# FasterDecoding/TEAL

Measured on AMD Instinct MI355X. Metric: decode tokens/sec (bs=1), Llama-2-7B fp16 @50% activation sparsity, higher is better.
Workload: dtype f16; 1 GPU; Llama-2-7B bs=1 decode, uniform 50% sparsity, hipGraph-captured step; mode=engine, parallelism=single GPU, context_positions=6..866

## Files before the change

### teal_amd/csrc/teal_sampler.hip

```cpp
#include "teal_common.h"

namespace teal {


template <bool BF16>
__device__ __forceinline__ void sample_full(const uint16_t* __restrict__ logits, const int V, const int top_k,
                                            const float inv_temp, unsigned long long* __restrict__ rng_state,
                                            int* __restrict__ token_out, int* __restrict__ pos_inout,
                                            int* __restrict__ history, const int history_len) {
    __shared__ unsigned int hist[256];
    __shared__ unsigned int whist[16][256];
    __shared__ float fred[16];
    __shared__ int ired[16];
    __shared__ unsigned int sel[2];
    __shared__ unsigned int suf[256];
    const int tid = threadIdx.x, lane = tid & 63, wave = tid >> 6;
    const bool filter = top_k > 0 && top_k < V;
    const int V8 = V >> 3;
    const u32x4* lv = reinterpret_cast<const u32x4*>(logits);
    uint32_t pivot_key = 0;
    float mx = -INFINITY;
    for (int i = tid; i < 16 * 256; i += 1024) (&whist[0][0])[i] = 0;
    __syncthreads();
    for (int i = tid; i < V8; i += 1024) {
        const u32x4 w = lv[i];
#pragma unroll
        for (int j = 0; j < 4; ++j) {
            const uint32_t lo = w[j] & 0xFFFFu, hi = w[j] >> 16;
            mx = fmaxf(mx, fmaxf(bits_to_float(lo, BF16), bits_to_float(hi, BF16)));
            if (filter) {
                atomicAdd(&whist[wave][order_key16(lo, BF16) >> 8], 1u);
                atomicAdd(&whist[wave][order_key16(hi, BF16) >> 8], 1u);
            }
        }
    }
    for (int i = (V8 << 3) + tid; i < V; i += 1024) {
        mx = fmaxf(mx, bits_to_float(logits[i], BF16));
        if (filter) atomicAdd(&whist[wave][order_key16(logits[i], BF16) >> 8], 1u);
    }
#pragma unroll
    for (int d = 32; d >= 1; d >>= 1) mx = fmaxf(mx, __shfl_xor(mx, d));
    if (lane == 0) fred[wave] = mx;
    __syncthreads();
    if (tid < 256) {
        unsigned int a = 0;
#pragma unroll
        for (int w = 0; w < 16; ++w) a += whist[w][tid];
        hist[tid] = a;
    }
    __syncthreads();
    mx = fred[0];
#pragma unroll
    for (int w = 1; w < 16; ++w) mx = fmaxf(mx, fred[w]);
    if (filter) {
        select_bin(hist, suf, sel, (unsigned int)top_k, tid);
        __syncthreads();
        const unsigned int hb = sel[0], need2 = sel[1];
        __syncthreads();
        for (int i = tid; i < 16 * 256; i += 1024) (&whist[0][0])[i] = 0;
        __syncthreads();
        for (int i = tid; i < V8; i += 1024) {
            const u32x4 w = lv[i];
#pragma unroll
            for (int j = 0; j < 4; ++j) {
                const uint32_t k0 = order_key16(w[j] & 0xFFFFu, BF16), k1 = order_key16(w[j] >> 16, BF16);
                if ((k0 >> 8) == hb) atomicAdd(&whist[wave][k0 & 0xFFu], 1u);
                if ((k1 >> 8) == hb) atomicAdd(&whist[wave][k1 & 0xFFu], 1u);
            }
        }
        for (int i = (V8 << 3) + tid; i < V; i += 1024) {
            const uint32_t k = order_key16(logits[i], BF16);
            if ((k >> 8) == hb) atomicAdd(&whist[wave][k & 0xFFu], 1u);
        }
        __syncthreads();
        if (tid < 256) {
            unsigned int a = 0;
#pragma unroll
            for (int w = 0; w < 16; ++w) a += whist[w][tid];
            hist[tid] = a;
        }
        __syncthreads();
        select_bin(hist, suf, sel, need2, tid);
        if (tid == 0) sel[0] = (hb << 8) | sel[0];
        __syncthreads();
        pivot_key = sel[0];
    }
    const uint32_t seed = (uint32_t)rng_state[0], ctr = (uint32_t)rng_state[1];
    float best = -1.0f;
    int besti = 0x7FFFFFFF;
    auto consider = [&](const uint32_t b, const int i) {
        if (filter && order_key16(b, BF16) < pivot_key) return;
        const float pnum = expf((bits_to_float(b, BF16) - mx) * inv_temp);
        const float u = ((float)(hash3(seed, ctr, (uint32_t)i) >> 8) + 0.5f) * (1.0f / 16777216.0f);
        const float scv = pnum / (-logf(u));
        if (scv > best || (scv == best && i < besti)) { best = scv; besti = i; }
    };
    for (int i = tid; i < V8; i += 1024) {
        const u32x4 w = lv[i];
#pragma unroll
        for (int j = 0; j < 4; ++j) {
            consider(w[j] & 0xFFFFu, i * 8 + 2 * j);
            consider(w[j] >> 16, i * 8 + 2 * j + 1);
        }
    }
    for (int i = (V8 << 3) + tid; i < V; i += 1024) consider(logits[i], i);
#pragma unroll
    for (int d = 32; d >= 1; d >>= 1) {
        const float ob = __shfl_xor(best, d);
        const int oi = __shfl_xor(besti, d);
        if (ob > best || (ob == best && oi < besti)) { best = ob; besti = oi; }
    }
    __syncthreads();
    if (lane == 0) { fred[wave] = best; ired[wave] = besti; }
    __syncthreads();
    if (tid == 0) {
        for (int w = 1; w < 16; ++w)
            if (fred[w] > best || (fred[w] == best && ired[w] < besti)) { best = fred[w]; besti = ired[w]; }
        token_out[0] = besti;
        const unsigned long long c = rng_state[1];
        if (history && (long long)c < (long long)history_len) history[c] = besti;
        rng_state[1] = c + 1ull;
        if (pos_inout) pos_inout[0] = pos_inout[0] + 1;
    }
}

template <bool BF16>
__global__ __launch_bounds__(1024) void sample_topk_kernel(const uint16_t* __restrict__ logits, const int V,
                                                            const int top_k, const float inv_temp,
                                                            unsigned long long* __restrict__ rng_state,
                                                            int* __restrict__ token_out, int* __restrict__ pos_inout,
                                                            int* __restrict__ history, const int history_len) {
    sample_full<BF16>(logits, V, top_k, inv_temp, rng_state, token_out, pos_inout, history, history_len);
}

__device__ __forceinline__ bool slot_off(const int* __restrict__ active, const int slot) { return !((active[0] >> slot) & 1); }

template <bool BF16>
__global__ __launch_bounds__(1024) void sample_topk_slot_kernel(const uint16_t* __restrict__ logits, const int V,
                                                                 const int top_k, const float inv_temp,
                                                                 unsigned long long* __restrict__ rng_state,
                                                                 int* __restrict__ token_out, int* __restrict__ pos_inout,
                                                                 int* __restrict__ history, const int history_len,
                                                                 const int* __restrict__ active, const int slot) {
    if (slot_off(active, slot)) return;
    sample_full<BF16>(logits, V, top_k, inv_temp, rng_state, token_out, pos_inout, history, history_len);
}


template <bool BF16, int NV>
__device__ __forceinline__ void sample_window_body(const uint16_t* __restrict__ logits, const int V, const int top_k, const float inv_temp,
                                                   unsigned long long* __restrict__ rng_state, int* __restrict__ token_out,
                                                   int* __restrict__ pos_inout, int* __restrict__ history, const int history_len,
                                                   unsigned long long* __restrict__ phase) {
    auto stamp_s = [&](const int i) { if (phase && threadIdx.x == 0) phase[i] = wall_clock64(); };
    stamp_s(0);
    __shared__ unsigned int hist[256];
    __shared__ unsigned int whist[16][256];
    __shared__ float fred[16];
    __shared__ int ired[16];
    __shared__ unsigned int sel[2];
    const int tid = threadIdx.x, lane = tid & 63, wave = tid >> 6;
    const bool filter = top_k > 0 && top_k < V;
    const int V8 = V >> 3;
    const u32x4* lv = reinterpret_cast<const u32x4*>(logits);
    u32x4 kv[NV];
#pragma unroll
    for (int v = 0; v < NV; ++v) kv[v] = lv[min(v * 1024 + tid, V8 - 1)];
    const unsigned long long seed64 = rng_state[0], ctr64 = rng_state[1];
    const int pos0 = pos_inout ? pos_inout[0] : 0;
    for (int i = tid; i < 16 * 256; i += 1024) (&whist[0][0])[i] = 0;
    uint32_t kmax = 0u;
#pragma unroll
    for (int v = 0; v < NV; ++v) {
        const bool ok = v * 1024 + tid < V8;
#pragma unroll
        for (int j = 0; j < 4; ++j) {
            const uint32_t k0 = order_key16(kv[v][j] & 0xFFFFu, BF16), k1 = order_key16(kv[v][j] >> 16, BF16);
            kv[v][j] = ok ? (k0 | (k1 << 16)) : 0u;
            kmax = ok ? max(kmax, max(k0, k1)) : kmax;
        }
    }
#pragma unroll
    for (int d = 32; d >= 1; d >>= 1) kmax = max(kmax, (uint32_t)__shfl_xor((int)kmax, d));
    if (lane == 0) ired[wave] = (int)kmax;
    __syncthreads();
    kmax = (uint32_t)ired[0];
#pragma unroll
    for (int w = 1; w < 16; ++w) kmax = max(kmax, (uint32_t)ired[w]);
    auto key_bits = [](const uint32_t k) -> uint32_t { return (k & 0x8000u) ? (k ^ 0x8000u) : (~k & 0xFFFFu); };
    const float mx = bits_to_float(key_bits(kmax), BF16);
    stamp_s(1);
    auto merge_hist = [&]() {
        __syncthreads();
        if (tid < 256) {
            unsigned int a = 0;
#pragma unroll
            for (int w = 0; w < 16; ++w) a += whist[w][tid];
            hist[tid] = a;
        }
        __syncthreads();
    };
    uint32_t pivot_key = 0u;
    if (filter) {
        for (int sh = BF16 ? 0 : 3;; sh += 3) {
            if (sh > 8) sh = 8;
#pragma unroll
            for (int v = 0; v < NV; ++v) {
                if (v * 1024 + tid < V8) {
#pragma unroll
                    for (int j = 0; j < 4; ++j) {
                        const uint32_t d0 = (kmax - (kv[v][j] & 0xFFFFu)) >> sh, d1 = (kmax - (kv[v][j] >> 16)) >> sh;
                        if (d0 < 256u) atomicAdd(&whist[wave][255u - d0], 1u);
                        if (d1 < 256u) atomicAdd(&whist[wave][255u - d1], 1u);
                    }
                }
            }
            merge_hist();
            unsigned int inwin = 0;
            {
                unsigned int a = (tid < 256) ? hist[tid] : 0u;
                a = (unsigned int)wave_sum_f((float)a);
                if (lane == 0) fred[wave] = (float)a;
                __syncthreads();
                inwin = (unsigned int)(fred[0] + fred[1] + fred[2] + fred[3]);
            }
            if (inwin >= (unsigned int)top_k || sh == 8) {
                select_bin(hist, nullptr, sel, (unsigned int)top_k, tid);
                const unsigned int d = 255u - sel[0], need2 = sel[1];
                __syncthreads();
                if (sh == 0) {
                    pivot_key = kmax - d;
                } else {
                    for (int i = tid; i < 16 * 256; i += 1024) (&whist[0][0])[i] = 0;
                    __syncthreads();
                    const uint32_t lowmask = (1u << sh) - 1u;
#pragma unroll
                    for (int v = 0; v < NV; ++v) {
                        if (v * 1024 + tid < V8) {
#pragma unroll
                            for (int j = 0; j < 4; ++j) {
                                const uint32_t e0 = kmax - (kv[v][j] & 0xFFFFu), e1 = kmax - (kv[v][j] >> 16);
                                if ((e0 >> sh) == d) atomicAdd(&whist[wave][255u - (e0 & lowmask)], 1u);
                                if ((e1 >> sh) == d) atomicAdd(&whist[wave][255u - (e1 & lowmask)], 1u);
                            }
                        }
                    }
                    merge_hist();
                    select_bin(hist, nullptr, sel, need2, tid);
                    pivot_key = kmax - ((d << sh) | (255u - sel[0]));
                    __syncthreads();
                }
                break;
            }
            for (int i = tid; i < 16 * 256; i += 1024) (&whist[0][0])[i] = 0;
            __syncthreads();
        }
    }
    stamp_s(2);
    const uint32_t seed = (uint32_t)seed64, ctr = (uint32_t)ctr64;
    float best = -1.0f;
    int besti = 0x7FFFFFFF;
    auto consider = [&](const uint32_t key, const int i) {
        if (key < pivot_key) return;
        const float pnum = expf((bits_to_float(key_bits(key), BF16) - mx) * inv_temp);
        const float u = ((float)(hash3(seed, ctr, (uint32_t)i) >> 8) + 0.5f) * (1.0f / 16777216.0f);
        const float scv = pnum / (-logf(u));
        if (scv > best || (scv == best && i < besti)) { best = scv; besti = i; }
    };
#pragma unroll
    for (int v = 0; v < NV; ++v) {
        const int i = v * 1024 + tid;
        if (i < V8) {
#pragma unroll
            for (int j = 0; j < 4; ++j) {
                consider(kv[v][j] & 0xFFFFu, i * 8 + 2 * j);
                consider(kv[v][j] >> 16, i * 8 + 2 * j + 1);
            }
        }
    }
    stamp_s(3);
#pragma unroll
    for (int d = 32; d >= 1; d >>= 1) {
        const float ob = __shfl_xor(best, d);
        const int oi = __shfl_xor(besti, d);
        if (ob > best || (ob == best && oi < besti)) { best = ob; besti = oi; }
    }
    __syncthreads();
    if (lane == 0) { fred[wave] = best; ired[wave] = besti; }
    __syncthreads();
    if (tid == 0) {
        for (int w = 1; w < 16; ++w)
            if (fred[w] > best || (fred[w] == best && ired[w] < besti)) { best = fred[w]; besti = ired[w]; }
        token_out[0] = besti;
        if (history && (long long)ctr64 < (long long)history_len) history[ctr64] = besti;
        rng_state[1] = ctr64 + 1ull;
        if (pos_inout) pos_inout[0] = pos0 + 1;
    }
    stamp_s(4);
}

template <bool BF16, int NV>
__global__ __launch_bounds__(1024) void sample_topk_window_kernel(const uint16_t* __restrict__ logits, const int V,
                                                                   const int top_k, const float inv_temp,
                                                                   unsigned long long* __restrict__ rng_state,
                                                                   int* __restrict__ token_out, int* __restrict__ pos_inout,
                                                                   int* __restrict__ history, const int history_len,
                                                                   unsigned long long* __restrict__ phase) {
    sample_window_body<BF16, NV>(logits, V, top_k, inv_temp, rng_state, token_out, pos_inout, history, history_len, phase);
}

template <bool BF16, int NV>
__global__ __launch_bounds__(1024) void sample_topk_window_slot_kernel(const uint16_t* __restrict__ logits, const int V,
                                                                        const int top_k, const float inv_temp,
                                                                        unsigned long long* __restrict__ rng_state,
                                                                        int* __restrict__ token_out, int* __restrict__ pos_inout,
                                                                        int* __restrict__ history, const int history_len,
                                                                        const int* __restrict__ active, const int slot) {
    if (slot_off(active, slot)) return;
    sample_window_body<BF16, NV>(logits, V, top_k, inv_temp, rng_state, token_out, pos_inout, history, history_len, nullptr);
}

template <bool BF16, int NK, bool COARSE = false>
__device__ __forceinline__ uint32_t window_pivot(const uint32_t (&keys)[NK], const uint32_t valid, const uint32_t kmax,
                                                 const unsigned int top_k, unsigned int* hist, unsigned int (*whist)[256],
                                                 float* fred, unsigned int* sel, const int tid) {
    const int lane = tid & 63, wave = tid >> 6;
    auto merge_hist = [&]() {
        __syncthreads();
        if (tid < 256) {
            unsigned int a = 0;
#pragma unroll
            for (int w = 0; w < 16; ++w) a += whist[w][tid];
            hist[tid] = a;
        }
        __syncthreads();
    };
    uint32_t pivot_key = 0u;
    for (int i = tid; i < 16 * 256; i += 1024) (&whist[0][0])[i] = 0;
    __syncthreads();
    for (int sh = BF16 ? 0 : 3;; sh += 3) {
        if (sh > 8) sh = 8;
#pragma unroll
        for (int j = 0; j < NK; ++j) {
            const uint32_t d = (kmax - keys[j]) >> sh;
            if (((valid >> j) & 1u) && d < 256u) atomicAdd(&whist[wave][255u - d], 1u);
        }
        merge_hist();
        unsigned int inwin = 0;
        {
            unsigned int a = (tid < 256) ? hist[tid] : 0u;
            a = (unsigned int)wave_sum_f((float)a);
            if (lane == 0) fred[wave] = (float)a;
            __syncthreads();
            inwin = (unsigned int)(fred[0] + fred[1] + fred[2] + fred[3]);
        }
        if (inwin >= top_k || sh == 8) {
            select_bin(hist, nullptr, sel, top_k, tid);
            const unsigned int d = 255u - sel[0], need2 = sel[1];
            __syncthreads();
            if (sh == 0) {
                pivot_key = kmax - d;
            } else if (COARSE) {
                const uint32_t span = ((d + 1u) << sh) - 1u;
                pivot_key = span >= kmax ? 0u : kmax - span;
            } else {
                for (int i = tid; i < 16 * 256; i += 1024) (&whist[0][0])[i] = 0;
                __syncthreads();
                const uint32_t lowmask = (1u << sh) - 1u;
#pragma unroll
                for (int j = 0; j < NK; ++j) {
                    const uint32_t e = kmax - keys[j];
                    if (((valid >> j) & 1u) && (e >> sh) == d) atomicAdd(&whist[wave][255u - (e & lowmask)], 1u);
                }
                merge_hist();
                select_bin(hist, nullptr, sel, need2, tid);
                pivot_key = kmax - ((d << sh) | (255u - sel[0]));
                __syncthreads();
            }
            break;
        }
        for (int i = tid; i < 16 * 256; i += 1024) (&whist[0][0])[i] = 0;
        __syncthreads();
    }
    return pivot_key;
}

__device__ __forceinline__ uint32_t block_max_u32(uint32_t v, int* ired, const int tid) {
    const int lane = tid & 63, wave = tid >> 6;
#pragma unroll
    for (int d = 32; d >= 1; d >>= 1) v = max(v, (uint32_t)__shfl_xor((int)v, d));
    __syncthreads();
    if (lane == 0) ired[wave] = (int)v;
    __syncthreads();
    v = (uint32_t)ired[0];
#pragma unroll
    for (int w = 1; w < 16; ++w) v = max(v, (uint32_t)ired[w]);
    return v;
}

template <bool BF16>
__device__ __forceinline__ void sample_multi_body(const uint16_t* __restrict__ logits, const int V, const int top_k, const float inv_temp,
                                                  unsigned long long* __restrict__ rng_state, int* __restrict__ token_out,
                                                  int* __restrict__ pos_inout, int* __restrict__ history, const int history_len,
                                                  unsigned char* __restrict__ slot) {
    __shared__ unsigned int hist[256];
    __shared__ unsigned int whist[16][256];
    __shared__ float fred[16];
    __shared__ int ired[16];
    __shared__ unsigned int sel[2];
    __shared__ unsigned int lcnt;
    __shared__ unsigned int lflag;
    __shared__ unsigned int gcount[kSampMaxGroups];
    const int tid = threadIdx.x, lane = tid & 63, wave = tid >> 6;
    const int g = blockIdx.x, G = gridDim.x;
    const int V8 = V >> 3;
    unsigned long long* cand = reinterpret_cast<unsigned long long*>(slot);
    unsigned int* counts = reinterpret_cast<unsigned int*>(slot + (size_t)kSampMaxGroups * kSampCap * 8);
    unsigned int* ticket = counts + kSampMaxGroups;
    const int vi = g * 1024 + tid;
    const bool ok = vi < V8;
    const u32x4 raw = reinterpret_cast<const u32x4*>(logits)[min(vi, V8 - 1)];
    const unsigned long long seed64 = rng_state[0], ctr64 = rng_state[1];
    const int pos0 = pos_inout ? pos_inout[0] : 0;
    if (tid == 0) lcnt = 0u;
    uint32_t keys[8];
    uint32_t kmax = 0u;
#pragma unroll
    for (int j = 0; j < 4; ++j) {
        keys[2 * j] = order_key16(raw[j] & 0xFFFFu, BF16);
        keys[2 * j + 1] = order_key16(raw[j] >> 16, BF16);
        if (ok) kmax = max(kmax, max(keys[2 * j], keys[2 * j + 1]));
    }
    kmax = block_max_u32(kmax, ired, tid);
    const unsigned int chunk_keys = (unsigned int)(min(V8 - g * 1024, 1024) * 8);
    const uint32_t lpivot = chunk_keys <= (unsigned int)top_k ? 0u
                            : window_pivot<BF16, 8, true>(keys, ok ? 0xFFu : 0u, kmax, (unsigned int)top_k, hist, whist, fred, sel, tid);
    __syncthreads();
    if (ok) {
#pragma unroll
        for (int j = 0; j < 8; ++j) {
            if (keys[j] >= lpivot) {
                const unsigned int s = atomicAdd(&lcnt, 1u);
                if (s < (unsigned int)kSampCap)
                    __hip_atomic_store(&cand[(size_t)g * kSampCap + s], ((unsigned long long)keys[j] << 32) | (unsigned int)(vi * 8 + j),
                                       __ATOMIC_RELAXED, __HIP_MEMORY_SCOPE_AGENT);
            }
        }
    }
    __syncthreads();
    if (tid == 0) __hip_atomic_store(&counts[g], lcnt, __ATOMIC_RELAXED, __HIP_MEMORY_SCOPE_AGENT);
    asm volatile("s_waitcnt vmcnt(0)" ::: "memory");
    __syncthreads();
    if (tid == 0) {
        const unsigned t = __hip_atomic_fetch_add(ticket, 1u, __ATOMIC_RELAXED, __HIP_MEMORY_SCOPE_AGENT);
        lflag = (t == (unsigned)G - 1u) ? 1u : 0u;
    }
    __syncthreads();
    if (lflag == 0u) return;
    if (tid == 0) __hip_atomic_store(ticket, 0u, __ATOMIC_RELAXED, __HIP_MEMORY_SCOPE_AGENT);
    constexpr int NC = kSampMaxGroups * kSampCap / 1024;
    unsigned long long craw[NC];
#pragma unroll
    for (int j = 0; j < NC; ++j) {
        const int sidx = j * 1024 + tid;
        craw[j] = sidx / kSampCap < G ? __hip_atomic_load(&cand[sidx], __ATOMIC_RELAXED, __HIP_MEMORY_SCOPE_AGENT) : 0ull;
    }
    if (tid < kSampMaxGroups) gcount[tid] = tid < G ? __hip_atomic_load(&counts[tid], __ATOMIC_RELAXED, __HIP_MEMORY_SCOPE_AGENT) : 0u;
    __syncthreads();
    bool overflow = false;
#pragma unroll
    for (int q = 0; q < kSampMaxGroups; ++q) overflow |= gcount[q] > (unsigned int)kSampCap;
    if (overflow) {
        sample_full<BF16>(logits, V, top_k, inv_temp, rng_state, token_out, pos_inout, history, history_len);
        return;
    }
    uint32_t ck[NC], ci[NC], cvalid = 0u;
    uint32_t gmax = 0u;
#pragma unroll
    for (int j = 0; j < NC; ++j) {
        const int sidx = j * 1024 + tid, gq = sidx / kSampCap, jj = sidx % kSampCap;
        ck[j] = 0u; ci[j] = 0u;
        if (gq < G && (unsigned int)jj < gcount[gq]) {
            ck[j] = (uint32_t)(craw[j] >> 32); ci[j] = (uint32_t)craw[j];
            cvalid |= 1u << j;
            gmax = max(gmax, ck[j]);
        }
    }
    gmax = block_max_u32(gmax, ired, tid);
    const uint32_t pivot = window_pivot<BF16, NC>(ck, cvalid, gmax, (unsigned int)top_k, hist, whist, fred, sel, tid);
    auto key_bits = [](const uint32_t k) -> uint32_t { return (k & 0x8000u) ? (k ^ 0x8000u) : (~k & 0xFFFFu); };
    const float mx = bits_to_float(key_bits(gmax), BF16);
    const uint32_t seed = (uint32_t)seed64, ctr = (uint32_t)ctr64;
    float best = -1.0f;
    int besti = 0x7FFFFFFF;
#pragma unroll
    for (int j = 0; j < NC; ++j) {
        if (((cvalid >> j) & 1u) && ck[j] >= pivot) {
            const int i = (int)ci[j];
            const float pnum = expf((bits_to_float(key_bits(ck[j]), BF16) - mx) * inv_temp);
            const float u = ((float)(hash3(seed, ctr, (uint32_t)i) >> 8) + 0.5f) * (1.0f / 16777216.0f);
            const float scv = pnum / (-logf(u));
            if (scv > best || (scv == best && i < besti)) { best = scv; besti = i; }
        }
    }
#pragma unroll
    for (int d = 32; d >= 1; d >>= 1) {
        const float ob = __shfl_xor(best, d);
        const int oi = __shfl_xor(besti, d);
        if (ob > best || (ob == best && oi < besti)) { best = ob; besti = oi; }
    }
    __syncthreads();
    if (lane == 0) { fred[wave] = best; ired[wave] = besti; }
    __syncthreads();
    if (tid == 0) {
        for (int w = 1; w < 16; ++w)
            if (fred[w] > best || (fred[w] == best && ired[w] < besti)) { best = fred[w]; besti = ired[w]; }
        token_out[0] = besti;
        if (history && (long long)ctr64 < (long long)history_len) history[ctr64] = besti;
        rng_state[1] = ctr64 + 1ull;
        if (pos_inout) pos_inout[0] = pos0 + 1;
    }
}

template <bool BF16>
__global__ __launch_bounds__(1024) void sample_topk_multi_kernel(const uint16_t* __restrict__ logits, const int V,
                                                                  const int top_k, const float inv_temp,
                                                                  unsigned long long* __restrict__ rng_state,
                                                                  int* __restrict__ token_out, int* __restrict__ pos_inout,
                                                                  int* __restrict__ history, const int history_len,
                                                                  unsigned char* __restrict__ slot) {
    sample_multi_body<BF16>(logits, V, top_k, inv_temp, rng_state, token_out, pos_inout, history, history_len, slot);
}

template <bool BF16>
__global__ __launch_bounds__(1024) void sample_topk_multi_slot_kernel(const uint16_t* __restrict__ logits, const int V,
                                                                       const int top_k, const float inv_temp,
                                                                       unsigned long long* __restrict__ rng_state,
                                                                       int* __restrict__ token_out, int* __restrict__ pos_inout,
                                                                       int* __restrict__ history, const int history_len,
                                                                       unsigned char* __restrict__ scratch, const int* __restrict__ active,
                                                                       const int slot) {
    if (slot_off(active, slot)) return;
    sample_multi_body<BF16>(logits, V, top_k, inv_temp, rng_state, token_out, pos_inout, history, history_len, scratch);
}

}

using namespace teal;

namespace {
int sample_launch(const void* logits, int vocab, int dtype, int top_k, float temperature, void* rng_state, int32_t* token_out,
                  int32_t* pos_inout, int32_t* history, int history_len, void* ws, size_t ws_bytes, const int32_t* active, int slot_id,
                  void* stream) {
    if (!logits || !rng_state || !token_out || vocab <= 0) return TEAL_ERR_ARG;
    if (dtype != TEAL_F16 && dtype != TEAL_BF16) return TEAL_ERR_DTYPE;
    if (!aligned16(logits)) return TEAL_ERR_ALIGN;
    const float inv_temp = 1.0f / fmaxf(temperature, 1e-5f);
    hipStream_t st = reinterpret_cast<hipStream_t>(stream);
    auto* lg = reinterpret_cast<const uint16_t*>(logits);
    auto* rs = reinterpret_cast<unsigned long long*>(rng_state);
#define TEAL_SAMPLE(KERNEL) hipLaunchKernelGGL((KERNEL), dim3(1), dim3(1024), 0, st, lg, vocab, top_k, inv_temp, rs, token_out, pos_inout, history, history_len)
#define TEAL_SAMPLE_W(KERNEL) hipLaunchKernelGGL((KERNEL), dim3(1), dim3(1024), 0, st, lg, vocab, top_k, inv_temp, rs, token_out, pos_inout, history, history_len, phase_start_only())
#define TEAL_SAMPLE_S(KERNEL) hipLaunchKernelGGL((KERNEL), dim3(1), dim3(1024), 0, st, lg, vocab, top_k, inv_temp, rs, token_out, pos_inout, history, history_len, active, slot_id)
    const bool bf = dtype == TEAL_BF16;
    if ((vocab & 7) == 0 && vocab > 8192 && vocab <= kSampMaxGroups * 8192 && top_k > 0 && top_k < vocab && ws_prepared(ws, ws_bytes)) {
        unsigned char* slot = ws_sampler(ws);
        const dim3 grid((vocab / 8 + 1023) / 1024), block(1024);
        if (active) {
            if (bf) hipLaunchKernelGGL((sample_topk_multi_slot_kernel<true>), grid, block, 0, st, lg, vocab, top_k, inv_temp, rs, token_out, pos_inout, history, history_len, slot, active, slot_id);
            else hipLaunchKernelGGL((sample_topk_multi_slot_kernel<false>), grid, block, 0, st, lg, vocab, top_k, inv_temp, rs, token_out, pos_inout, history, history_len, slot, active, slot_id);
        } else {
            if (bf) hipLaunchKernelGGL((sample_topk_multi_kernel<true>), grid, block, 0, st, lg, vocab, top_k, inv_temp, rs, token_out, pos_inout, history, history_len, slot);
            else hipLaunchKernelGGL((sample_topk_multi_kernel<false>), grid, block, 0, st, lg, vocab, top_k, inv_temp, rs, token_out, pos_inout, history, history_len, slot);
        }
    } else if ((vocab & 7) == 0 && vocab <= 4 * 8192) {
        if (active) { if (bf) TEAL_SAMPLE_S((sample_topk_window_slot_kernel<true, 4>)); else TEAL_SAMPLE_S((sample_topk_window_slot_kernel<false, 4>)); }
        else if (bf) TEAL_SAMPLE_W((sample_topk_window_kernel<true, 4>)); else TEAL_SAMPLE_W((sample_topk_window_kernel<false, 4>));
    } else if ((vocab & 7) == 0 && vocab <= 16 * 8192) {
        if (active) { if (bf) TEAL_SAMPLE_S((sample_topk_window_slot_kernel<true, 16>)); else TEAL_SAMPLE_S((sample_topk_window_slot_kernel<false, 16>)); }
        else if (bf) TEAL_SAMPLE_W((sample_topk_window_kernel<true, 16>)); else TEAL_SAMPLE_W((sample_topk_window_kernel<false, 16>));
    } else {
        if (active) { if (bf) TEAL_SAMPLE_S((sample_topk_slot_kernel<true>)); else TEAL_SAMPLE_S((sample_topk_slot_kernel<false>)); }
        else if (bf) TEAL_SAMPLE((sample_topk_kernel<true>)); else TEAL_SAMPLE((sample_topk_kernel<false>));
    }
#undef TEAL_SAMPLE
#undef TEAL_SAMPLE_W
#undef TEAL_SAMPLE_S
    return hipGetLastError() == hipSuccess ? TEAL_OK : TEAL_ERR_LAUNCH;
}
}

extern "C" {

int teal_sample_topk_ws(const void* logits, int vocab, int dtype, int top_k, float temperature, void* rng_state,
                        int32_t* token_out, int32_t* pos_inout, int32_t* history, int history_len, void* ws, size_t ws_bytes,
                        void* stream) {
    return sample_launch(logits, vocab, dtype, top_k, temperature, rng_state, token_out, pos_inout, history, history_len, ws, ws_bytes,
                         nullptr, 0, stream);
}

int teal_sample_topk_slot(const void* logits, int vocab, int dtype, int top_k, float temperature, void* rng_state, int32_t* token_out,
                          int32_t* pos_inout, int32_t* history, int history_len, void* ws, size_t ws_bytes, const int32_t* active, int slot,
                          void* stream) {
    if (!active || slot < 0 || slot > 31) return TEAL_ERR_ARG;
    return sample_launch(logits, vocab, dtype, top_k, temperature, rng_state, token_out, pos_inout, history, history_len, ws, ws_bytes,
                         active, slot, stream);
}

int teal_sample_topk(const void* logits, int vocab, int dtype, int top_k, float temperature, void* rng_state,
                     int32_t* token_out, int32_t* pos_inout, int32_t* history, int history_len, void* stream) {
    return teal_sample_topk_ws(logits, vocab, dtype, top_k, temperature, rng_state, token_out, pos_inout, history, history_len,
                               nullptr, 0, stream);
}

}
```

Before: 548.7 tokens/s.

## Restructure multi-block top-k sampler with DPP reductions and wave-level selection

Rewrites the multi-block top-k sampler. Block max and argmax now use DPP row reductions, bin selection uses a single-wave suffix-scan select over a padded wide histogram, and candidates are compacted with ballot-based ranks instead of a shared atomic counter. The last block detects overflow through the ticket counter and reads each group's max from the packed count word, so it can usually skip the two-level window pivot. It also adds optional diagnostic timestamps. The goal is fewer barriers and atomics in a per-token kernel, at the cost of more intricate code and a larger shared-memory footprint.

```diff
diff --git a/teal_amd/csrc/teal_sampler.hip b/teal_amd/csrc/teal_sampler.hip
--- a/teal_amd/csrc/teal_sampler.hip
+++ b/teal_amd/csrc/teal_sampler.hip
@@ -320,7 +320,69 @@
     sample_window_body<BF16, NV>(logits, V, top_k, inv_temp, rng_state, token_out, pos_inout, history, history_len, nullptr);
 }
 
-template <bool BF16, int NK, bool COARSE = false>
+constexpr int kSelPitch = 65;
+constexpr int kSelWide = 64;
+constexpr int kSelWords = kSelWide * kSelPitch;
+template <int R>
+__device__ __forceinline__ unsigned int sel_slot(const unsigned int b) { return (b % R) * kSelPitch + b / R; }
+
+template <int CTRL>
+__device__ __forceinline__ int dpp_row(const int old, const int v) { return __builtin_amdgcn_update_dpp(old, v, CTRL, 0xf, 0xf, false); }
+__device__ __forceinline__ uint32_t wave_max_u32(uint32_t v) {
+    v = max(v, (uint32_t)dpp_row<0x111>((int)v, (int)v));
+    v = max(v, (uint32_t)dpp_row<0x112>((int)v, (int)v));
+    v = max(v, (uint32_t)dpp_row<0x114>((int)v, (int)v));
+    v = max(v, (uint32_t)dpp_row<0x118>((int)v, (int)v));
+    return max(max((uint32_t)__builtin_amdgcn_readlane((int)v, 15), (uint32_t)__builtin_amdgcn_readlane((int)v, 31)),
+               max((uint32_t)__builtin_amdgcn_readlane((int)v, 47), (uint32_t)__builtin_amdgcn_readlane((int)v, 63)));
+}
+__device__ __forceinline__ int wave_min_i32(int v) {
+    v = min(v, dpp_row<0x111>(v, v));
+    v = min(v, dpp_row<0x112>(v, v));
+    v = min(v, dpp_row<0x114>(v, v));
+    v = min(v, dpp_row<0x118>(v, v));
+    return min(min(__builtin_amdgcn_readlane(v, 15), __builtin_amdgcn_readlane(v, 31)),
+               min(__builtin_amdgcn_readlane(v, 47), __builtin_amdgcn_readlane(v, 63)));
+}
+__device__ __forceinline__ unsigned int wave_suffix_sum(unsigned int v, const int lane) {
+    v += (unsigned int)dpp_row<0x101>(0, (int)v);
+    v += (unsigned int)dpp_row<0x102>(0, (int)v);
+    v += (unsigned int)dpp_row<0x104>(0, (int)v);
+    v += (unsigned int)dpp_row<0x108>(0, (int)v);
+    const unsigned int t1 = (unsigned int)__builtin_amdgcn_readlane((int)v, 16), t2 = (unsigned int)__builtin_amdgcn_readlane((int)v, 32),
+                       t3 = (unsigned int)__builtin_amdgcn_readlane((int)v, 48);
+    const int row = lane >> 4;
+    return v + (row == 0 ? t1 + t2 + t3 : row == 1 ? t2 + t3 : row == 2 ? t3 : 0u);
+}
+__device__ __forceinline__ void wave_argmax(float& best, int& besti) {
+    const float m = wave_max_f(best);
+    besti = wave_min_i32(best == m ? besti : 0x7FFFFFFF);
+    best = m;
+}
+
+template <int R>
+__device__ __forceinline__ void wave_select(const unsigned int* hist, unsigned int* sel, const unsigned int need, const int tid) {
+    if (tid < 64) {
+        unsigned int own = 0;
+#pragma unroll
+        for (int r = 0; r < R; ++r) own += hist[r * kSelPitch + tid];
+        const unsigned int incl = wave_suffix_sum(own, tid), above = incl - own;
+        const unsigned int total = (unsigned int)__builtin_amdgcn_readlane((int)incl, 0);
+        const unsigned long long m = __ballot(above < need && incl >= need);
+        if (m == 0ull) {
+            if (tid == 0) { sel[0] = 0u; sel[1] = need; sel[2] = total; }
+        } else {
+            const int L = __ffsll((long long)m) - 1;
+            const unsigned int aboveL = (unsigned int)__builtin_amdgcn_readlane((int)above, L);
+            const unsigned int h = tid < R ? hist[tid * kSelPitch + L] : 0u;
+            const unsigned int a = aboveL + wave_suffix_sum(h, tid) - h;
+            if (a < need && a + h >= need) { sel[0] = (unsigned int)(R * L + tid); sel[1] = need - a; sel[2] = total; }
+        }
+    }
+    __syncthreads();
+}
+
+template <bool BF16, int NK>
 __device__ __forceinline__ uint32_t window_pivot(const uint32_t (&keys)[NK], const uint32_t valid, const uint32_t kmax,
                                                  const unsigned int top_k, unsigned int* hist, unsigned int (*whist)[256],
                                                  float* fred, unsigned int* sel, const int tid) {
@@ -360,9 +422,6 @@
             __syncthreads();
             if (sh == 0) {
                 pivot_key = kmax - d;
-            } else if (COARSE) {
-                const uint32_t span = ((d + 1u) << sh) - 1u;
-                pivot_key = span >= kmax ? 0u : kmax - span;
             } else {
                 for (int i = tid; i < 16 * 256; i += 1024) (&whist[0][0])[i] = 0;
                 __syncthreads();
@@ -385,35 +444,27 @@
     return pivot_key;
 }
 
-__device__ __forceinline__ uint32_t block_max_u32(uint32_t v, int* ired, const int tid) {
-    const int lane = tid & 63, wave = tid >> 6;
-#pragma unroll
-    for (int d = 32; d >= 1; d >>= 1) v = max(v, (uint32_t)__shfl_xor((int)v, d));
-    __syncthreads();
-    if (lane == 0) ired[wave] = (int)v;
-    __syncthreads();
-    v = (uint32_t)ired[0];
-#pragma unroll
-    for (int w = 1; w < 16; ++w) v = max(v, (uint32_t)ired[w]);
-    return v;
-}
+constexpr int kSampPhaseRow = 32, kSampPhaseB = 8;
 
 template <bool BF16>
 __device__ __forceinline__ void sample_multi_body(const uint16_t* __restrict__ logits, const int V, const int top_k, const float inv_temp,
                                                   unsigned long long* __restrict__ rng_state, int* __restrict__ token_out,
                                                   int* __restrict__ pos_inout, int* __restrict__ history, const int history_len,
-                                                  unsigned char* __restrict__ slot) {
-    __shared__ unsigned int hist[256];
+                                                  unsigned char* __restrict__ slot, unsigned long long* __restrict__ phase) {
+    __shared__ unsigned int hist[kSelWords];
     __shared__ unsigned int whist[16][256];
     __shared__ float fred[16];
     __shared__ int ired[16];
-    __shared__ unsigned int sel[2];
-    __shared__ unsigned int lcnt;
+    __shared__ unsigned int sel[3];
+    __shared__ unsigned int wcnts[16];
     __shared__ unsigned int lflag;
-    __shared__ unsigned int gcount[kSampMaxGroups];
     const int tid = threadIdx.x, lane = tid & 63, wave = tid >> 6;
     const int g = blockIdx.x, G = gridDim.x;
     const int V8 = V >> 3;
+    auto stamp = [&](const int i) {
+        if (kDiagnostics && phase && tid == 0) phase[g * kSampPhaseRow + i] = wall_clock64();
+    };
+    stamp(0);
     unsigned long long* cand = reinterpret_cast<unsigned long long*>(slot);
     unsigned int* counts = reinterpret_cast<unsigned int*>(slot + (size_t)kSampMaxGroups * kSampCap * 8);
     unsigned int* ticket = counts + kSampMaxGroups;
@@ -422,7 +473,7 @@
     const u32x4 raw = reinterpret_cast<const u32x4*>(logits)[min(vi, V8 - 1)];
     const unsigned long long seed64 = rng_state[0], ctr64 = rng_state[1];
     const int pos0 = pos_inout ? pos_inout[0] : 0;
-    if (tid == 0) lcnt = 0u;
+    for (int i = tid; i < kSelWords; i += 1024) hist[i] = 0u;
     uint32_t keys[8];
     uint32_t kmax = 0u;
 #pragma unroll
@@ -431,63 +482,115 @@
         keys[2 * j + 1] = order_key16(raw[j] >> 16, BF16);
         if (ok) kmax = max(kmax, max(keys[2 * j], keys[2 * j + 1]));
     }
-    kmax = block_max_u32(kmax, ired, tid);
+    kmax = wave_max_u32(kmax);
+    if (lane == 0) ired[wave] = (int)kmax;
+    __syncthreads();
+    kmax = (uint32_t)ired[0];
+#pragma unroll
+    for (int w = 1; w < 16; ++w) kmax = max(kmax, (uint32_t)ired[w]);
+    stamp(1);
     const unsigned int chunk_keys = (unsigned int)(min(V8 - g * 1024, 1024) * 8);
-    const uint32_t lpivot = chunk_keys <= (unsigned int)top_k ? 0u
-                            : window_pivot<BF16, 8, true>(keys, ok ? 0xFFu : 0u, kmax, (unsigned int)top_k, hist, whist, fred, sel, tid);
-    __syncthreads();
-    if (ok) {
-#pragma unroll
-        for (int j = 0; j < 8; ++j) {
-            if (keys[j] >= lpivot) {
-                const unsigned int s = atomicAdd(&lcnt, 1u);
-                if (s < (unsigned int)kSampCap)
-                    __hip_atomic_store(&cand[(size_t)g * kSampCap + s], ((unsigned long long)keys[j] << 32) | (unsigned int)(vi * 8 + j),
-                                       __ATOMIC_RELAXED, __HIP_MEMORY_SCOPE_AGENT);
-            }
-        }
-    }
-    __syncthreads();
-    if (tid == 0) __hip_atomic_store(&counts[g], lcnt, __ATOMIC_RELAXED, __HIP_MEMORY_SCOPE_AGENT);
+    uint32_t lpivot = 0u;
+    if (chunk_keys > (unsigned int)top_k) {
+        for (int sh = BF16 ? 0 : 3;; sh += 3) {
+            if (sh > 8) sh = 8;
+            if (ok) {
+#pragma unroll
+                for (int j = 0; j < 8; ++j) {
+                    const uint32_t d = (kmax - keys[j]) >> sh;
+                    if (d < 256u) atomicAdd(&hist[sel_slot<4>(255u - d)], 1u);
+                }
+            }
+            __syncthreads();
+            wave_select<4>(hist, sel, (unsigned int)top_k, tid);
+            const unsigned int d = 255u - sel[0], inwin = sel[2];
+            if (tid < 4 * kSelPitch) hist[tid] = 0u;
+            if (inwin >= (unsigned int)top_k || sh == 8) {
+                const uint32_t span = ((d + 1u) << sh) - 1u;
+                lpivot = span >= kmax ? 0u : kmax - span;
+                break;
+            }
+            __syncthreads();
+        }
+    }
+    stamp(2);
+    uint32_t rank[8], cmask = 0u, wcnt = 0u;
+#pragma unroll
+    for (int j = 0; j < 8; ++j) {
+        const bool c = ok && keys[j] >= lpivot;
+        const unsigned long long m = __ballot(c);
+        rank[j] = wcnt + (uint32_t)lane_rank(m);
+        wcnt += (uint32_t)__popcll(m);
+        cmask |= c ? 1u << j : 0u;
+    }
+    if (lane == 0) wcnts[wave] = wcnt;
+    __syncthreads();
+    unsigned int cbase = 0u, ctotal = 0u;
+#pragma unroll
+    for (int w = 0; w < 16; ++w) {
+        const unsigned int c = wcnts[w];
+        cbase += w < wave ? c : 0u;
+        ctotal += c;
+    }
+#pragma unroll
+    for (int j = 0; j < 8; ++j) {
+        const unsigned int s = cbase + rank[j];
+        if (((cmask >> j) & 1u) && s < (unsigned int)kSampCap)
+            __hip_atomic_store(&cand[(size_t)g * kSampCap + s], ((unsigned long long)keys[j] << 32) | (unsigned int)(vi * 8 + j),
+                               __ATOMIC_RELAXED, __HIP_MEMORY_SCOPE_AGENT);
+    }
+    if (tid == 0) __hip_atomic_store(&counts[g], (kmax << 16) | ctotal, __ATOMIC_RELAXED, __HIP_MEMORY_SCOPE_AGENT);
     asm volatile("s_waitcnt vmcnt(0)" ::: "memory");
     __syncthreads();
     if (tid == 0) {
-        const unsigned t = __hip_atomic_fetch_add(ticket, 1u, __ATOMIC_RELAXED, __HIP_MEMORY_SCOPE_AGENT);
-        lflag = (t == (unsigned)G - 1u) ? 1u : 0u;
-    }
-    __syncthreads();
-    if (lflag == 0u) return;
+        const unsigned int over = ctotal > (unsigned int)kSampCap ? 1u : 0u;
+        const unsigned int t = __hip_atomic_fetch_add(ticket, 1u + (over << 16), __ATOMIC_RELAXED, __HIP_MEMORY_SCOPE_AGENT);
+        lflag = (t & 0xFFFFu) == (unsigned)G - 1u ? 1u + (((t >> 16) + over) ? 2u : 0u) : 0u;
+    }
+    __syncthreads();
+    stamp(3);
+    const unsigned int fl = lflag;
+    if (fl == 0u) return;
+    stamp(kSampPhaseB + 0);
     if (tid == 0) __hip_atomic_store(ticket, 0u, __ATOMIC_RELAXED, __HIP_MEMORY_SCOPE_AGENT);
+    if (fl & 2u) {
+        sample_full<BF16>(logits, V, top_k, inv_temp, rng_state, token_out, pos_inout, history, history_len);
+        return;
+    }
     constexpr int NC = kSampMaxGroups * kSampCap / 1024;
+    static_assert(1024 % kSampCap == 0 && 1024 / kSampCap == 2, "slot j of a thread belongs to chunk 2 j + (tid >> 9)");
     unsigned long long craw[NC];
+    unsigned int cw[kSampMaxGroups];
+#pragma unroll
+    for (int q = 0; q < kSampMaxGroups; ++q) cw[q] = q < G ? __hip_atomic_load(&counts[q], __ATOMIC_RELAXED, __HIP_MEMORY_SCOPE_AGENT) : 0u;
 #pragma unroll
     for (int j = 0; j < NC; ++j) {
         const int sidx = j * 1024 + tid;
         craw[j] = sidx / kSampCap < G ? __hip_atomic_load(&cand[sidx], __ATOMIC_RELAXED, __HIP_MEMORY_SCOPE_AGENT) : 0ull;
     }
-    if (tid < kSampMaxGroups) gcount[tid] = tid < G ? __hip_atomic_load(&counts[tid], __ATOMIC_RELAXED, __HIP_MEMORY_SCOPE_AGENT) : 0u;
-    __syncthreads();
-    bool overflow = false;
-#pragma unroll
-    for (int q = 0; q < kSampMaxGroups; ++q) overflow |= gcount[q] > (unsigned int)kSampCap;
-    if (overflow) {
-        sample_full<BF16>(logits, V, top_k, inv_temp, rng_state, token_out, pos_inout, history, history_len);
-        return;
-    }
+    uint32_t gmax = 0u;
+#pragma unroll
+    for (int q = 0; q < kSampMaxGroups; ++q) gmax = max(gmax, cw[q] >> 16);
     uint32_t ck[NC], ci[NC], cvalid = 0u;
-    uint32_t gmax = 0u;
+    const unsigned int odd = 0u - (unsigned int)(tid >> 9);
 #pragma unroll
     for (int j = 0; j < NC; ++j) {
-        const int sidx = j * 1024 + tid, gq = sidx / kSampCap, jj = sidx % kSampCap;
+        const unsigned int cnt = ((cw[2 * j] & ~odd) | (cw[2 * j + 1] & odd)) & 0xFFFFu;
         ck[j] = 0u; ci[j] = 0u;
-        if (gq < G && (unsigned int)jj < gcount[gq]) {
+        if ((unsigned int)(tid & (kSampCap - 1)) < cnt) {
             ck[j] = (uint32_t)(craw[j] >> 32); ci[j] = (uint32_t)craw[j];
             cvalid |= 1u << j;
-            gmax = max(gmax, ck[j]);
-        }
-    }
-    gmax = block_max_u32(gmax, ired, tid);
-    const uint32_t pivot = window_pivot<BF16, NC>(ck, cvalid, gmax, (unsigned int)top_k, hist, whist, fred, sel, tid);
+            const uint32_t d = gmax - ck[j];
+            if (d < (uint32_t)(64 * kSelWide)) atomicAdd(&hist[sel_slot<kSelWide>((uint32_t)(64 * kSelWide - 1) - d)], 1u);
+        }
+    }
+    stamp(kSampPhaseB + 1);
+    __syncthreads();
+    wave_select<kSelWide>(hist, sel, (unsigned int)top_k, tid);
+    uint32_t pivot;
+    if (sel[2] >= (unsigned int)top_k) pivot = gmax - ((uint32_t)(64 * kSelWide - 1) - sel[0]);
+    else pivot = window_pivot<BF16, NC>(ck, cvalid, gmax, (unsigned int)top_k, hist, whist, fred, sel, tid);
+    stamp(kSampPhaseB + 2);
     auto key_bits = [](const uint32_t k) -> uint32_t { return (k & 0x8000u) ? (k ^ 0x8000u) : (~k & 0xFFFFu); };
     const float mx = bits_to_float(key_bits(gmax), BF16);
     const uint32_t seed = (uint32_t)seed64, ctr = (uint32_t)ctr64;
@@ -503,23 +606,27 @@
             if (scv > best || (scv == best && i < besti)) { best = scv; besti = i; }
         }
     }
-#pragma unroll
-    for (int d = 32; d >= 1; d >>= 1) {
-        const float ob = __shfl_xor(best, d);
-        const int oi = __shfl_xor(besti, d);
-        if (ob > best || (ob == best && oi < besti)) { best = ob; besti = oi; }
-    }
-    __syncthreads();
+    wave_argmax(best, besti);
+    stamp(kSampPhaseB + 3);
     if (lane == 0) { fred[wave] = best; ired[wave] = besti; }
     __syncthreads();
     if (tid == 0) {
-        for (int w = 1; w < 16; ++w)
-            if (fred[w] > best || (fred[w] == best && ired[w] < besti)) { best = fred[w]; besti = ired[w]; }
+        float fw[16];
+        int iw[16];
+#pragma unroll
+        for (int w = 1; w < 16; ++w) { fw[w] = fred[w]; iw[w] = ired[w]; }
+#pragma unroll
+        for (int w = 1; w < 16; ++w) {
+            const bool t = fw[w] > best || (fw[w] == best && iw[w] < besti);
+            best = t ? fw[w] : best;
+            besti = t ? iw[w] : besti;
+        }
         token_out[0] = besti;
         if (history && (long long)ctr64 < (long long)history_len) history[ctr64] = besti;
         rng_state[1] = ctr64 + 1ull;
         if (pos_inout) pos_inout[0] = pos0 + 1;
     }
+    stamp(kSampPhaseB + 4);
 }
 
 template <bool BF16>
@@ -528,8 +635,8 @@
                                                                   unsigned long long* __restrict__ rng_state,
                                                                   int* __restrict__ token_out, int* __restrict__ pos_inout,
                                                                   int* __restrict__ history, const int history_len,
-                                                                  unsigned char* __restrict__ slot) {
-    sample_multi_body<BF16>(logits, V, top_k, inv_temp, rng_state, token_out, pos_inout, history, history_len, slot);
+                                                                  unsigned char* __restrict__ slot, unsigned long long* __restrict__ phase) {
+    sample_multi_body<BF16>(logits, V, top_k, inv_temp, rng_state, token_out, pos_inout, history, history_len, slot, phase);
 }
 
 template <bool BF16>
@@ -541,7 +648,7 @@
                                                                        unsigned char* __restrict__ scratch, const int* __restrict__ active,
                                                                        const int slot) {
     if (slot_off(active, slot)) return;
-    sample_multi_body<BF16>(logits, V, top_k, inv_temp, rng_state, token_out, pos_inout, history, history_len, scratch);
+    sample_multi_body<BF16>(logits, V, top_k, inv_temp, rng_state, token_out, pos_inout, history, history_len, scratch, nullptr);
 }
 
 }
@@ -570,8 +677,8 @@
             if (bf) hipLaunchKernelGGL((sample_topk_multi_slot_kernel<true>), grid, block, 0, st, lg, vocab, top_k, inv_temp, rs, token_out, pos_inout, history, history_len, slot, active, slot_id);
             else hipLaunchKernelGGL((sample_topk_multi_slot_kernel<false>), grid, block, 0, st, lg, vocab, top_k, inv_temp, rs, token_out, pos_inout, history, history_len, slot, active, slot_id);
         } else {
-            if (bf) hipLaunchKernelGGL((sample_topk_multi_kernel<true>), grid, block, 0, st, lg, vocab, top_k, inv_temp, rs, token_out, pos_inout, history, history_len, slot);
-            else hipLaunchKernelGGL((sample_topk_multi_kernel<false>), grid, block, 0, st, lg, vocab, top_k, inv_temp, rs, token_out, pos_inout, history, history_len, slot);
+            if (bf) hipLaunchKernelGGL((sample_topk_multi_kernel<true>), grid, block, 0, st, lg, vocab, top_k, inv_temp, rs, token_out, pos_inout, history, history_len, slot, phase_start_only());
+            else hipLaunchKernelGGL((sample_topk_multi_kernel<false>), grid, block, 0, st, lg, vocab, top_k, inv_temp, rs, token_out, pos_inout, history, history_len, slot, phase_start_only());
         }
     } else if ((vocab & 7) == 0 && vocab <= 4 * 8192) {
         if (active) { if (bf) TEAL_SAMPLE_S((sample_topk_window_slot_kernel<true, 4>)); else TEAL_SAMPLE_S((sample_topk_window_slot_kernel<false, 4>)); }
```

After: 549.8 tokens/s, median of 6. About the same (+0.2%).
